# teoremma/pgen-rs

Hardware: AMD Instinct MI355X
Metric: genotypes decoded/sec (variants x samples / s) (higher is better)
Workload: dtype u8

## Files before the change

pgen_rs_amd/csrc/gt_rowpick.hip:

```cpp
#include "gt_common.hip.h"
#include "kernels.h"

namespace pgenhip {

namespace {

constexpr int kThreads = 256;
constexpr int kWaves = kThreads / 64;
constexpr uint32_t kSegSamples = kScanSegmentSamples;
constexpr uint32_t kTilesPerSeg = 4;
constexpr uint32_t kStageBytes = kSegSamples / 4u;

typedef uint32_t v4u __attribute__((ext_vector_type(4)));

__device__ __forceinline__ uint64_t sgpr64_(uint64_t v)
{
    return ((uint64_t)(uint32_t)__builtin_amdgcn_readfirstlane((uint32_t)(v >> 32)) << 32) | (uint64_t)(uint32_t)__builtin_amdgcn_readfirstlane((uint32_t)v);
}

__host__ __device__ inline uint32_t table_bytes(uint32_t K) { return (2u * (K + 8u) + 15u) & ~15u; }
__host__ __device__ inline uint32_t rank_bytes(uint32_t n_seg) { return (4u * (n_seg + 1u) + 15u) & ~15u; }
__host__ __device__ inline uint32_t codes_bytes(uint32_t K) { return ((K + 3u) / 4u + 16u + 15u) & ~15u; }

template <bool HAS_VIDX, bool COMPACT>
__global__ __launch_bounds__(kThreads) void gt_rowpick_kernel(EmitArgs a, ScanArgs sc, uint32_t n_seg)
{
    extern __shared__ __attribute__((aligned(16))) uint8_t s_mem[];
    const uint32_t K = a.kept_count;
    uint16_t *const s_idx = reinterpret_cast<uint16_t *>(s_mem);
    uint32_t *const s_rank = reinterpret_cast<uint32_t *>(s_mem + table_bytes(K));
    const uint32_t tid = threadIdx.x;
    const uint32_t lane = tid & 63u;
    const uint32_t wave = __builtin_amdgcn_readfirstlane(tid >> 6);
    uint8_t *const stage = s_mem + table_bytes(K) + rank_bytes(n_seg) + wave * (kStageBytes + codes_bytes(K));
    uint8_t *const codes = stage + kStageBytes;

    for (uint32_t r = tid; r < K + 8u; r += (uint32_t)kThreads)
        s_idx[r] = r < K ? (uint16_t)(a.kept_idx[r] & (kSegSamples - 1u)) : (uint16_t)0;
    for (uint32_t g = tid; g <= n_seg; g += (uint32_t)kThreads) s_rank[g] = sc.seg_rank[g];
    for (uint32_t i = lane; i < codes_bytes(K); i += 64u) codes[i] = 0;
    __syncthreads();

    const uint32_t R = a.record_size;
    const uint64_t wave_step = (uint64_t)gridDim.x * kWaves;
    const uint64_t j0 = (uint64_t)blockIdx.x * kWaves + wave;
    if (j0 >= (uint64_t)a.n_variants) return;
    const uint64_t rows = ((uint64_t)a.n_variants - j0 + wave_step - 1ull) / wave_step;
    const uint64_t pieces = rows * n_seg;

    const uint32_t tail_t = (R - 1u) >> 10;
    const uint32_t tail_b = tail_t * 1024u + lane * 16u;
    const uint32_t tail_off = min(tail_b, R - 16u);
    const uint32_t tail_shift = tail_b + 16u <= R ? 0u : min(tail_b - (R - 16u), 16u);
    const bool lines = !COMPACT && a.line_off != nullptr;

    auto load_piece = [&](uint64_t row, uint32_t seg, v4u(&dst)[kTilesPerSeg]) {
        const uint8_t *__restrict__ rec = HAS_VIDX ? gathered_record(a, row) : a.records + row * a.record_stride;
        const uint32_t tile0 = seg * kTilesPerSeg;
        const uint8_t *__restrict__ sub = rec + (uint64_t)tile0 * 1024u;
#pragma unroll
        for (uint32_t t = 0; t < kTilesPerSeg; t++) {
            const uint8_t *src16 = tile0 + t < tail_t ? sub + lane * 16u + t * 1024u : rec + tail_off;
            __builtin_memcpy(&dst[t], src16, 16);
        }
    };
    auto pick_piece = [&](uint32_t seg, const v4u(&w)[kTilesPerSeg]) {
        const uint32_t tile0 = seg * kTilesPerSeg;
#pragma unroll
        for (uint32_t tile = 0; tile < kTilesPerSeg; tile++) {
            v4u x = w[tile];
            if (tile0 + tile == tail_t && tail_shift != 0u) {
                uint64_t lo = (uint64_t)x.x | ((uint64_t)x.y << 32), hi = (uint64_t)x.z | ((uint64_t)x.w << 32);
                const uint32_t sh8 = tail_shift * 8u;
                if (sh8 >= 128u) { lo = 0ull; hi = 0ull; }
                else if (sh8 >= 64u) { lo = hi >> (sh8 - 64u); hi = 0ull; }
                else { lo = (lo >> sh8) | (hi << (64u - sh8)); hi >>= sh8; }
                x = v4u{(uint32_t)lo, (uint32_t)(lo >> 32), (uint32_t)hi, (uint32_t)(hi >> 32)};
            }
            if (tile0 + tile <= tail_t) *reinterpret_cast<v4u *>(stage + tile * 1024u + lane * 16u) = x;
        }
        __builtin_amdgcn_fence(__ATOMIC_RELEASE, "wavefront");
        __builtin_amdgcn_wave_barrier();
        __builtin_amdgcn_fence(__ATOMIC_ACQUIRE, "wavefront");
        const uint32_t k0 = __builtin_amdgcn_readfirstlane(s_rank[seg]);
        const uint32_t k1 = __builtin_amdgcn_readfirstlane(s_rank[seg + 1u]);
        const uint32_t cb0 = k0 >> 2, cb1 = (k1 + 3u) >> 2;
#pragma clang loop unroll(disable)
        for (uint32_t b = cb0 + lane; b < cb1 && k0 < k1; b += 64u) {
            uint32_t byte = 0u;
#pragma unroll
            for (uint32_t j = 0; j < 4u; j++) {
                const uint32_t r = 4u * b + j;
                const bool mine = r >= k0 && r < k1;
                const uint32_t s16 = s_idx[mine ? r : k0];
                const uint32_t code = ((uint32_t)stage[s16 >> 2] >> ((s16 & 3u) * 2u)) & 3u;
                byte |= (mine ? code : 0u) << (2u * j);
            }
            if (b == cb0 && (k0 & 3u) != 0u) byte |= codes[b];
            codes[b] = (uint8_t)byte;
        }
        __builtin_amdgcn_fence(__ATOMIC_RELEASE, "wavefront");
        __builtin_amdgcn_wave_barrier();
    };
    uint64_t L_lo = 0ull, L_po = 0ull, L_po1 = 0ull, C_lo = 0ull, C_po = 0ull, C_plen = 0ull, P_lo = 0ull, P_po = 0ull, P_plen = 0ull;
    uint32_t C_pfx = 0u, P_pfx = 0u;
    auto load_offsets = [&](uint64_t row) {
        if (lines) {
            L_lo = a.line_off[row];
            L_po = a.prefix_off[row];
            L_po1 = a.prefix_off[row + 1ull];
        }
    };
    auto load_prefix = [&]() {
        if (lines) {
            C_lo = sgpr64_(L_lo);
            C_po = sgpr64_(L_po);
            C_plen = sgpr64_(L_po1) - C_po;
            C_pfx = lane < C_plen ? (uint32_t)a.prefix_blob[C_po + lane] : 0u;
        }
    };
    auto emit_row = [&](uint64_t row) {
        __builtin_amdgcn_fence(__ATOMIC_ACQUIRE, "wavefront");
        if (COMPACT) {
            uint8_t *const crow = a.out + row * a.out_stride;
            const uint32_t len = (K + 3u) >> 2;
            const uint32_t head = min((16u - ((uint32_t)(uintptr_t)crow & 15u)) & 15u, len);
            const uint32_t n_chunks = (len - head) >> 4;
            for (uint32_t c = lane; c < n_chunks; c += 64u) {
                v4u v;
                __builtin_memcpy(&v, codes + head + (c << 4), 16);
                *reinterpret_cast<v4u *>(crow + head + (c << 4)) = v;
            }
            const uint32_t tail_off = head + (n_chunks << 4);
            const uint32_t off = lane < 16u ? lane : tail_off + (lane - 16u);
            if (lane < 16u ? lane < head : (lane < 32u && off < len)) crow[off] = codes[off];
            __builtin_amdgcn_fence(__ATOMIC_RELEASE, "wavefront");
            __builtin_amdgcn_wave_barrier();
            return;
        }
        uint8_t *row_out;
        if (lines) {
            uint64_t lo = P_lo, p0 = P_po, plen = P_plen;
            if (n_seg < 2u) {
                p0 = a.prefix_off[row];
                plen = a.prefix_off[row + 1ull] - p0;
                lo = a.line_off[row];
            }
            uint8_t *const line = a.out + lo;
            if (n_seg >= 2u && lane < plen) line[lane] = (uint8_t)P_pfx;
            for (uint64_t i = (n_seg >= 2u ? 64ull : 0ull) + lane; i < plen; i += 64ull) line[i] = a.prefix_blob[p0 + i];
            row_out = line + plen;
        } else {
            row_out = a.out + row * a.out_stride;
        }
        const uint8_t *cd = codes;
        flush_text4<2>(
            [cd](auto c0, uint32_t g, uint32_t &k0, uint32_t &k1, uint32_t &k2, uint32_t &k3) {
                constexpr uint32_t C0 = decltype(c0)::value;
                const uint32_t win = C0 == 0u ? (uint32_t)cd[g] : (uint32_t)cd[g] | ((uint32_t)cd[g + 1u] << 8);
                k0 = __builtin_amdgcn_ubfe(win, 2u * C0, 2u);
                k1 = __builtin_amdgcn_ubfe(win, 2u * C0 + 2u, 2u);
                k2 = __builtin_amdgcn_ubfe(win, 2u * C0 + 4u, 2u);
                k3 = __builtin_amdgcn_ubfe(win, 2u * C0 + 6u, 2u);
            },
            [cd](uint32_t r) -> uint32_t { return ((uint32_t)cd[r >> 2] >> ((r & 3u) * 2u)) & 3u; },
            0u, row_out, 0ull, 4ull * K + 1ull, 0u, K, lane, sc.align_stores != 0u);
        __builtin_amdgcn_fence(__ATOMIC_RELEASE, "wavefront");
        __builtin_amdgcn_wave_barrier();
    };
    auto landed = [&](const v4u(&w)[kTilesPerSeg]) {
#pragma unroll
        for (uint32_t t = 0; t < kTilesPerSeg; t++) asm volatile("" ::"v"(w[t].x), "v"(w[t].y), "v"(w[t].z), "v"(w[t].w));
    };

    v4u b0[kTilesPerSeg], b1[kTilesPerSeg];
    uint64_t row = j0, nrow = j0;
    uint32_t seg = 0u, nseg = 0u;
    auto advance = [&](uint64_t &r, uint32_t &s) {
        if (++s == n_seg) { s = 0u; r += wave_step; }
    };
    bool pending = false;
    uint64_t pending_row = 0ull;
    auto issue_next = [&](uint64_t p, v4u(&dst)[kTilesPerSeg]) {
        advance(nrow, nseg);
        const bool real = p + 1ull < pieces;
        if (real && nseg == 0u) load_offsets(nrow);
        if (real && nseg == 1u) load_prefix();
        load_piece(real ? nrow : row, real ? nseg : seg, dst);
    };
    auto finish_piece = [&]() {
        if (seg + 1u == n_seg) {
            pending = true;
            pending_row = row;
            P_lo = C_lo; P_po = C_po; P_plen = C_plen; P_pfx = C_pfx;
        }
        advance(row, seg);
    };
    load_offsets(nrow);
    load_piece(nrow, nseg, b0);
    for (uint64_t p = 0;;) {
        landed(b0);
        if (pending) { emit_row(pending_row); pending = false; }
        issue_next(p, b1);
        pick_piece(seg, b0);
        finish_piece();
        if (++p == pieces) break;
        landed(b1);
        if (pending) { emit_row(pending_row); pending = false; }
        issue_next(p, b0);
        pick_piece(seg, b1);
        finish_piece();
        if (++p == pieces) break;
    }
    if (pending) emit_row(pending_row);
}

}

bool gt_rowpick_applicable(const EmitArgs &a, int num_cus)
{
    const uint32_t n_seg = (a.sample_count + kSegSamples - 1u) / kSegSamples;
    return a.kept_idx != nullptr && a.kept_count >= 1u && a.kept_count <= kRowPickMaxKept && a.record_size >= 16u && n_seg >= 1u && n_seg <= 4096u &&
           (uint64_t)a.n_variants >= 8ull * (uint64_t)num_cus * kWaves;
}

namespace {

struct RowPickLaunch {
    void (*kern)(EmitArgs, ScanArgs, uint32_t);
    uint32_t n_seg, lds, max_blocks;
};

bool plan(const EmitArgs &a, const Tuning &t, int num_cus, bool compact, RowPickLaunch &L)
{
    if (a.kept_idx == nullptr || a.kept_count > kRowPickMaxKept) return false;
    L.n_seg = (a.sample_count + kSegSamples - 1u) / kSegSamples;
    if (L.n_seg < 1u || L.n_seg > 4096u || a.record_size < 16u) return false;
    L.lds = table_bytes(a.kept_count) + rank_bytes(L.n_seg) + (uint32_t)kWaves * (kStageBytes + codes_bytes(a.kept_count));
    const bool g = gathered(a);
    if (compact) L.kern = g ? gt_rowpick_kernel<true, true> : gt_rowpick_kernel<false, true>;
    else L.kern = g ? gt_rowpick_kernel<true, false> : gt_rowpick_kernel<false, false>;
    int per_cu = 0;
    if (hipOccupancyMaxActiveBlocksPerMultiprocessor(&per_cu, L.kern, kThreads, L.lds) != hipSuccess || per_cu < 1) per_cu = 1;
    const int want = t.rowpick_blocks_per_cu > 0 ? t.rowpick_blocks_per_cu : (!compact && a.sample_count < 24576u ? 4 : 2);
    if (want < per_cu) per_cu = want;
    L.max_blocks = (uint32_t)per_cu * (uint32_t)num_cus;
    return true;
}

}

uint32_t gt_rowpick_resident_waves(const EmitArgs &a, const Tuning &t, int num_cus, bool compact)
{
    RowPickLaunch L;
    return plan(a, t, num_cus, compact, L) ? L.max_blocks * (uint32_t)kWaves : 0u;
}

hipError_t launch_gt_rowpick(const EmitArgs &a, const ScanArgs &sc, const Tuning &t, int num_cus, hipStream_t stream, bool compact)
{
    if (a.n_variants == 0) return hipSuccess;
    RowPickLaunch L;
    if (!plan(a, t, num_cus, compact, L)) return hipErrorInvalidValue;
    const uint64_t need = ((uint64_t)a.n_variants + kWaves - 1ull) / kWaves;
    hipLaunchKernelGGL(L.kern, dim3((uint32_t)(need < L.max_blocks ? need : L.max_blocks)), dim3(kThreads), L.lds, stream, a, sc, L.n_seg);
    return hipGetLastError();
}

}
```

Measured before the change: 1472 billion.

## Load records from aligned window base with nontemporal loads instead of tail shifting

Record loads now start from a 16-byte-aligned base below each record and walk fixed-size windows, using nontemporal 16-byte loads clamped to the last aligned chunk. This removes the per-tile tail shift logic. The misalignment offset is folded into the LDS lookup with a wrap mask, and kept-sample splits between windows are recomputed with a ballot over samples that spill into the next window. The number of windows per row can differ from the segment count, which adds per-window split logic and the risk of off-by-one errors at window boundaries.

```diff
diff --git a/pgen_rs_amd/csrc/gt_rowpick.hip b/pgen_rs_amd/csrc/gt_rowpick.hip
--- a/pgen_rs_amd/csrc/gt_rowpick.hip
+++ b/pgen_rs_amd/csrc/gt_rowpick.hip
@@ -45,45 +45,50 @@
     const uint64_t wave_step = (uint64_t)gridDim.x * kWaves;
     const uint64_t j0 = (uint64_t)blockIdx.x * kWaves + wave;
     if (j0 >= (uint64_t)a.n_variants) return;
-    const uint64_t rows = ((uint64_t)a.n_variants - j0 + wave_step - 1ull) / wave_step;
-    const uint64_t pieces = rows * n_seg;
-
-    const uint32_t tail_t = (R - 1u) >> 10;
-    const uint32_t tail_b = tail_t * 1024u + lane * 16u;
-    const uint32_t tail_off = min(tail_b, R - 16u);
-    const uint32_t tail_shift = tail_b + 16u <= R ? 0u : min(tail_b - (R - 16u), 16u);
+
     const bool lines = !COMPACT && a.line_off != nullptr;
 
-    auto load_piece = [&](uint64_t row, uint32_t seg, v4u(&dst)[kTilesPerSeg]) {
-        const uint8_t *__restrict__ rec = HAS_VIDX ? gathered_record(a, row) : a.records + row * a.record_stride;
-        const uint32_t tile0 = seg * kTilesPerSeg;
-        const uint8_t *__restrict__ sub = rec + (uint64_t)tile0 * 1024u;
-#pragma unroll
-        for (uint32_t t = 0; t < kTilesPerSeg; t++) {
-            const uint8_t *src16 = tile0 + t < tail_t ? sub + lane * 16u + t * 1024u : rec + tail_off;
-            __builtin_memcpy(&dst[t], src16, 16);
-        }
-    };
-    auto pick_piece = [&](uint32_t seg, const v4u(&w)[kTilesPerSeg]) {
-        const uint32_t tile0 = seg * kTilesPerSeg;
-#pragma unroll
-        for (uint32_t tile = 0; tile < kTilesPerSeg; tile++) {
-            v4u x = w[tile];
-            if (tile0 + tile == tail_t && tail_shift != 0u) {
-                uint64_t lo = (uint64_t)x.x | ((uint64_t)x.y << 32), hi = (uint64_t)x.z | ((uint64_t)x.w << 32);
-                const uint32_t sh8 = tail_shift * 8u;
-                if (sh8 >= 128u) { lo = 0ull; hi = 0ull; }
-                else if (sh8 >= 64u) { lo = hi >> (sh8 - 64u); hi = 0ull; }
-                else { lo = (lo >> sh8) | (hi << (64u - sh8)); hi >>= sh8; }
-                x = v4u{(uint32_t)lo, (uint32_t)(lo >> 32), (uint32_t)hi, (uint32_t)(hi >> 32)};
-            }
-            if (tile0 + tile <= tail_t) *reinterpret_cast<v4u *>(stage + tile * 1024u + lane * 16u) = x;
-        }
+    struct Walk {
+        uint64_t row;
+        const uint8_t *base;
+        uint32_t d, n_win, win, last;
+    };
+    auto open_row = [&](uint64_t row) {
+        const uint64_t off = sgpr64_(HAS_VIDX ? gathered_offset(a, row) : row * a.record_stride);
+        Walk w;
+        w.row = row;
+        w.d = ((uint32_t)(uintptr_t)a.records + (uint32_t)off) & 15u;
+        w.base = a.records + (int64_t)(off - w.d);
+        w.n_win = (w.d + R + kStageBytes - 1u) / kStageBytes;
+        w.win = 0u;
+        w.last = (w.d + R - 1u) & ~15u;
+        return w;
+    };
+    const uint32_t lane16 = lane * 16u;
+    auto load_piece = [&](const Walk &w, v4u(&dst)[kTilesPerSeg]) {
+#pragma unroll
+        for (uint32_t t = 0; t < kTilesPerSeg; t++) dst[t] = load_nt16(w.base + min(w.win * kStageBytes + t * 1024u + lane16, w.last));
+    };
+    auto split = [&](uint32_t p, uint32_t d) -> uint32_t {
+        if (p > n_seg) return K;
+        const uint32_t hi = __builtin_amdgcn_readfirstlane(s_rank[p]);
+        if (d == 0u) return hi;
+        const uint32_t cnt = hi - (uint32_t)__builtin_amdgcn_readfirstlane(s_rank[p - 1u]);
+        const bool late = lane < cnt && (uint32_t)s_idx[lane < cnt ? hi - 1u - lane : 0u] >= kSegSamples - 4u * d;
+        return hi - (uint32_t)__builtin_popcountll(__builtin_amdgcn_ballot_w64(late));
+    };
+    uint32_t k_prev = 0u;
+    auto pick_piece = [&](const Walk &c, const v4u(&w)[kTilesPerSeg]) {
+        const uint32_t d = c.d;
+#pragma unroll
+        for (uint32_t tile = 0; tile < kTilesPerSeg; tile++)
+            if (c.win * kStageBytes + tile * 1024u < d + R) *reinterpret_cast<v4u *>(stage + tile * 1024u + lane16) = w[tile];
         __builtin_amdgcn_fence(__ATOMIC_RELEASE, "wavefront");
         __builtin_amdgcn_wave_barrier();
         __builtin_amdgcn_fence(__ATOMIC_ACQUIRE, "wavefront");
-        const uint32_t k0 = __builtin_amdgcn_readfirstlane(s_rank[seg]);
-        const uint32_t k1 = __builtin_amdgcn_readfirstlane(s_rank[seg + 1u]);
+        const uint32_t k0 = c.win == 0u ? 0u : k_prev;
+        const uint32_t k1 = split(c.win + 1u, d);
+        k_prev = k1;
         const uint32_t cb0 = k0 >> 2, cb1 = (k1 + 3u) >> 2;
 #pragma clang loop unroll(disable)
         for (uint32_t b = cb0 + lane; b < cb1 && k0 < k1; b += 64u) {
@@ -93,7 +98,7 @@
                 const uint32_t r = 4u * b + j;
                 const bool mine = r >= k0 && r < k1;
                 const uint32_t s16 = s_idx[mine ? r : k0];
-                const uint32_t code = ((uint32_t)stage[s16 >> 2] >> ((s16 & 3u) * 2u)) & 3u;
+                const uint32_t code = ((uint32_t)stage[((s16 >> 2) + d) & (kStageBytes - 1u)] >> ((s16 & 3u) * 2u)) & 3u;
                 byte |= (mine ? code : 0u) << (2u * j);
             }
             if (b == cb0 && (k0 & 3u) != 0u) byte |= codes[b];
@@ -119,7 +124,7 @@
             C_pfx = lane < C_plen ? (uint32_t)a.prefix_blob[C_po + lane] : 0u;
         }
     };
-    auto emit_row = [&](uint64_t row) {
+    auto emit_row = [&](uint64_t row, uint32_t n_win) {
         __builtin_amdgcn_fence(__ATOMIC_ACQUIRE, "wavefront");
         if (COMPACT) {
             uint8_t *const crow = a.out + row * a.out_stride;
@@ -141,14 +146,14 @@
         uint8_t *row_out;
         if (lines) {
             uint64_t lo = P_lo, p0 = P_po, plen = P_plen;
-            if (n_seg < 2u) {
+            if (n_win < 2u) {
                 p0 = a.prefix_off[row];
                 plen = a.prefix_off[row + 1ull] - p0;
                 lo = a.line_off[row];
             }
             uint8_t *const line = a.out + lo;
-            if (n_seg >= 2u && lane < plen) line[lane] = (uint8_t)P_pfx;
-            for (uint64_t i = (n_seg >= 2u ? 64ull : 0ull) + lane; i < plen; i += 64ull) line[i] = a.prefix_blob[p0 + i];
+            if (n_win >= 2u && lane < plen) line[lane] = (uint8_t)P_pfx;
+            for (uint64_t i = (n_win >= 2u ? 64ull : 0ull) + lane; i < plen; i += 64ull) line[i] = a.prefix_blob[p0 + i];
             row_out = line + plen;
         } else {
             row_out = a.out + row * a.out_stride;
@@ -174,45 +179,46 @@
     };
 
     v4u b0[kTilesPerSeg], b1[kTilesPerSeg];
-    uint64_t row = j0, nrow = j0;
-    uint32_t seg = 0u, nseg = 0u;
-    auto advance = [&](uint64_t &r, uint32_t &s) {
-        if (++s == n_seg) { s = 0u; r += wave_step; }
-    };
+    Walk n = open_row(j0), c = n;
     bool pending = false;
     uint64_t pending_row = 0ull;
-    auto issue_next = [&](uint64_t p, v4u(&dst)[kTilesPerSeg]) {
-        advance(nrow, nseg);
-        const bool real = p + 1ull < pieces;
-        if (real && nseg == 0u) load_offsets(nrow);
-        if (real && nseg == 1u) load_prefix();
-        load_piece(real ? nrow : row, real ? nseg : seg, dst);
+    uint32_t pending_win = 0u;
+    auto issue_next = [&](v4u(&dst)[kTilesPerSeg]) -> bool {
+        bool real = true;
+        if (n.win + 1u < n.n_win) n.win++;
+        else if (n.row + wave_step < (uint64_t)a.n_variants) n = open_row(n.row + wave_step);
+        else real = false;
+        if (real && n.win == 0u) load_offsets(n.row);
+        if (real && n.win == 1u) load_prefix();
+        load_piece(n, dst);
+        return real;
     };
     auto finish_piece = [&]() {
-        if (seg + 1u == n_seg) {
+        if (c.win + 1u == c.n_win) {
             pending = true;
-            pending_row = row;
+            pending_row = c.row;
+            pending_win = c.n_win;
             P_lo = C_lo; P_po = C_po; P_plen = C_plen; P_pfx = C_pfx;
         }
-        advance(row, seg);
-    };
-    load_offsets(nrow);
-    load_piece(nrow, nseg, b0);
-    for (uint64_t p = 0;;) {
+        c = n;
+    };
+    load_offsets(n.row);
+    load_piece(n, b0);
+    for (;;) {
         landed(b0);
-        if (pending) { emit_row(pending_row); pending = false; }
-        issue_next(p, b1);
-        pick_piece(seg, b0);
+        if (pending) { emit_row(pending_row, pending_win); pending = false; }
+        bool more = issue_next(b1);
+        pick_piece(c, b0);
         finish_piece();
-        if (++p == pieces) break;
+        if (!more) break;
         landed(b1);
-        if (pending) { emit_row(pending_row); pending = false; }
-        issue_next(p, b0);
-        pick_piece(seg, b1);
+        if (pending) { emit_row(pending_row, pending_win); pending = false; }
+        more = issue_next(b0);
+        pick_piece(c, b1);
         finish_piece();
-        if (++p == pieces) break;
+        if (!more) break;
     }
-    if (pending) emit_row(pending_row);
+    if (pending) emit_row(pending_row, pending_win);
 }
 
 }
```

Result: no change. 1471 billion (-0.1%).
